# autonomousvision/volsurfs

Measured on AMD Instinct MI355X. Metric: Mrays/s (fwd+bwd) at 800x800, K=5 shells, higher is better.
Workload: dtype f16 (hash features, MLP on MFMA, composite: as the reference), f32 accumulate and I/O

## Files before the change

include/volsurfs_hip.h:

```cpp
#ifndef VOLSURFS_HIP_H
#define VOLSURFS_HIP_H

#include <stdint.h>

#ifdef __cplusplus
extern "C" {
#endif

#define VSA_OK 0
#define VSA_ERR_ARG (-1)
#define VSA_ERR_UNSUPPORTED (-2)

#define VSA_MAX_SHELLS 16

int vsa_version(void);

int vsa_composite_dense_fwd(const float* surfs_rgb, const float* surfs_alpha,
                            const float* rgb_bg, int bg_is_broadcast, float* out_rgb,
                            float* out_rgb_fg, float* out_bg_transmittance, float* out_weights,
                            float* out_surfs_rgb_h, float* out_surfs_alpha_h, int nr_rays,
                            int nr_shells, int carry_f16, void* stream);

int vsa_composite_dense_bwd(const float* surfs_rgb, const float* surfs_alpha,
                            const float* rgb_bg, int bg_is_broadcast, const float* g_rgb,
// ... 92 lines not shown
  void* balance;
  int32_t row_format;
  int32_t grads_zeroed;
  int32_t shared_rgb;
  int32_t shared_alpha;
} vsa_nt_plan;

long long vsa_nt_balance_bytes(void);
int vsa_nt_rebalance(const vsa_nt_plan* plan, void* stream);

int vsa_nt_mark(const vsa_nt_plan* plan, const int32_t* hit_slot, const float* hit_uv,
                const float* face_uvs, int nr_rays, float* tex_uv, uint8_t* marks, void* stream);

int vsa_nt_compact_frame(const vsa_nt_plan* plan, uint8_t* marks, int32_t* slot_of,
                         int32_t* texel_of_slot, float* slot_xy, int32_t* seg_start,
                         int32_t* block_scratch, void* stream);

int vsa_nt_encode_fwd(const vsa_nt_plan* plan, const void* tables_h, const float* slot_xy,
                      const int32_t* seg_start, void* features, void* stream);

int vsa_nt_mlp_fwd(const vsa_nt_plan* plan, const void* weights_h, const void* features,
                   const int32_t* seg_start, uint8_t* texels, void* pre_out, void* stream);

int vsa_nt_encode_mlp_fwd(const vsa_nt_plan* plan, const void* tables_h, const void* weights_h,
                          const float* slot_xy, const int32_t* seg_start, void* features,
                          uint8_t* texels, void* pre_out, void* stream);

int vsa_nt_mlp_bwd(const vsa_nt_plan* plan, const void* weights_h, void* features,
                   const int32_t* seg_start, uint16_t* grad_rows, float* grad_weights,
                   float* dfeat_abs_sum, float weight_grad_scale, void* stream);

int vsa_nt_shade_fwd(const vsa_nt_plan* plan, const int32_t* hit_slot, const float* tex_uv,
                     const float* rays_d, const float* tris, const int32_t* slot_of,
                     const int32_t* seg_start, const uint8_t* texels, int nr_rays,
                     float* surfs_rgb, float* surfs_alpha,
                     float* surfs_normals, float* coeffs_out, float* act_out, void* stream);

int vsa_nt_shade_bwd(const vsa_nt_plan* plan, const int32_t* hit_slot, const float* tex_uv,
                     const float* rays_d, const float* tris, const int32_t* slot_of,
                     const int32_t* seg_start, const uint8_t* texels, int nr_rays,
                     const float* g_surfs_rgb,
                     const float* g_surfs_alpha, float grad_scale, uint16_t* grad_rows,
                     const float* act_in, void* stream);

long long vsa_nt_planes_bytes(const vsa_nt_plan* plan);
int vsa_nt_export_planes(const vsa_nt_plan* plan, const int32_t* slot_of, const int32_t* seg_start,
                         const uint8_t* texels, uint8_t* planes, long long planes_bytes, void* stream);
int vsa_nt_import_planes(const vsa_nt_plan* plan, const uint8_t* planes, long long planes_bytes,
                         const int32_t* slot_of, const int32_t* seg_start, uint8_t* texels, void* stream);

int vsa_nt_encode_bwd(const vsa_nt_plan* plan, const void* dfeatures, const float* dfeat_abs_sum,
                      float grad_scale, const float* slot_xy, const int32_t* seg_start,
                      float* grad_tables, void* stream);

int vsa_nt_encode_bwd_range(const vsa_nt_plan* plan, const void* dfeatures,
                            const float* dfeat_abs_sum, float grad_scale, const float* slot_xy,
                            const int32_t* seg_start, float* grad_tables, int shell_begin,
                            int shell_end, void* stream);

typedef struct vsa_dp_flags vsa_dp_flags;
int vsa_dp_flags_create(int n, vsa_dp_flags** out);
int vsa_dp_flags_destroy(vsa_dp_flags* flags);
int vsa_dp_flags_read(const vsa_dp_flags* flags, uint32_t* host_out);

int vsa_nt_encode_bwd_phased(const vsa_nt_plan* plan, const void* dfeatures,
                             const float* dfeat_abs_sum, float grad_scale, const float* slot_xy,
                             const int32_t* seg_start, float* grad_tables, int n_phases,
                             const int32_t* phase_shell_end, vsa_dp_flags* flags, uint32_t* counters,
                             const uint32_t* epoch, int reserve_cus, void* stream);

int vsa_dp_signal(vsa_dp_flags* flags, int index, uint32_t* epoch, int advance_epoch, void* stream);

int vsa_dp_stream_wait(vsa_dp_flags* flags, int index, uint32_t value, int mode, void* stream);

#define VSA_GRID_MAX_LEVELS 32
typedef struct vsa_grid_plan {
  int32_t n_dims;
  int32_t n_levels;
  int32_t n_features;
  int32_t reserved0;
  float level_scale[VSA_GRID_MAX_LEVELS];
  int32_t level_res[VSA_GRID_MAX_LEVELS];
  int32_t level_size[VSA_GRID_MAX_LEVELS];
  int32_t level_offset[VSA_GRID_MAX_LEVELS + 1];
} vsa_grid_plan;

int vsa_grid_encode_fwd(const vsa_grid_plan* plan, const float* tables, const float* x,
                        int nr_points, float* out, void* stream);
int vsa_grid_encode_bwd(const vsa_grid_plan* plan, const float* x, const float* g_out,
                        int nr_points, float* grad_tables, void* stream);
int vsa_grid_encode_bwd_sliced(const vsa_grid_plan* plan, const float* x, const float* g_out,
                               int nr_points, float* grad_tables, float* workspace, void* stream);
int vsa_grid_encode_bwd_binned_workspace(const vsa_grid_plan* plan, int nr_points,
                                         long long* workspace_floats);
int vsa_grid_encode_bwd_binned(const vsa_grid_plan* plan, const float* x, const float* g_out,
                               int nr_points, float* grad_tables, float* workspace, void* stream);
int vsa_grid_encode_fwd_ld(const vsa_grid_plan* plan, const float* tables, const float* x,
                           int nr_points, float* out, int out_stride, int append_x, void* stream);
int vsa_grid_encode_bwd_ld(const vsa_grid_plan* plan, const float* x, const float* g_out,
                           int g_stride, int nr_points, float* grad_tables, void* stream);
int vsa_grid_encode_bwd_sliced_ld(const vsa_grid_plan* plan, const float* x, const float* g_out,
                                  int g_stride, int nr_points, float* grad_tables, float* workspace,
                                  void* stream);
int vsa_grid_encode_bwd_binned_ld(const vsa_grid_plan* plan, const float* x, const float* g_out,
                                  int g_stride, int nr_points, float* grad_tables, float* workspace,
                                  void* stream);
// ... 551 lines not shown
```

volsurfs_amd/csrc/nt_common.h:

```cpp
#pragma once
#include "common.h"

typedef _Float16 half2_t __attribute__((ext_vector_type(2)));
typedef _Float16 half4_t __attribute__((ext_vector_type(4)));
typedef _Float16 half8_t __attribute__((ext_vector_type(8)));
typedef float float16_t __attribute__((ext_vector_type(16)));

#define NT_DOM_BLOCK 4096

#define NT_FBLOCK 256
__device__ __forceinline__ long long nt_feat_index(const vsa_nt_plan& p, int type, int level,
                                                   int slot) {
  const long long blocks = p.slot_capacity / NT_FBLOCK;
  return (((long long)type * blocks + (slot >> 8)) * p.n_levels + level) * NT_FBLOCK + (slot & 255);
}
__device__ __forceinline__ long long nt_feat_plane_base(const vsa_nt_plan& p, int type, int level) {
  return ((long long)type * (p.slot_capacity / NT_FBLOCK) * p.n_levels + level) * NT_FBLOCK;
}
__device__ __forceinline__ long long nt_feat_in_plane(int n_levels, int slot) {
  return (long long)(slot >> 8) * (n_levels * NT_FBLOCK) + (slot & 255);
}

__host__ __device__ inline int nt_tex_index(int shell, int type, int deg) {
  return (shell * 2 + type) * VSA_NT_MAX_DEG + deg;
// ... 206 lines not shown
    begin = seg_start[sd];
    end = seg_start[sd + 1];
  }
  act = act && end > begin;
  const int units = act ? (end - begin + UNIT - 1) / UNIT : 0;
  const unsigned long long act_mask = __ballot(act);
  const long long pieces = __popcll(act_mask);
  if (pieces == 0) return;
  auto lane_cost = [&](int pl) { return act ? ovh * 16 + units * wt(pl, deg, wtype) : 0; };
  auto plane_cost = [&](int pl) -> long long {
    return (long long)(unsigned)__builtin_amdgcn_readlane(nt_wave_incl_scan(lane_cost(pl)), 63);
  };
  long long total = 0;
  for (int pl = 0; pl < n_planes; ++pl) total += plane_cost(pl);
  long long lo, hi;
  nt_split_range(plan, bal_id, total, lo, hi);
  if (hi <= lo) return;
  long long c0 = 0;
  for (int pl = 0; pl < n_planes && c0 < hi; ++pl) {
    const int cl = lane_cost(pl);
    const int incl = nt_wave_incl_scan(cl);
    const long long pc = (long long)(unsigned)__builtin_amdgcn_readlane(incl, 63);
    if (c0 + pc <= lo) {
      c0 += pc;
      continue;
    }
    const long long t0l = c0 + (long long)(incl - cl) + (long long)ovh * 16;
    const int w = wt(pl, deg, wtype);
    const long long span = (long long)units * w;
    bool hit = act && t0l < hi;
    int ua = 0, ub = 0;
    if (hit) {
      const long long a = lo > t0l ? lo - t0l : 0, b = hi - t0l < span ? hi - t0l : span;
      hit = b > a;
      if (hit) {
        ua = (int)(((unsigned)a + (unsigned)w - 1u) / (unsigned)w);
        ub = (int)(((unsigned)b + (unsigned)w - 1u) / (unsigned)w);
        hit = ub > ua;
      }
    }
    unsigned long long todo = __ballot(hit);
    while (todo) {
      const int j = __ffsll((long long)todo) - 1;
      todo &= todo - 1;
      const int jb = __builtin_amdgcn_readlane(begin, j), je = __builtin_amdgcn_readlane(end, j);
      const int ja = __builtin_amdgcn_readlane(ua, j), jub = __builtin_amdgcn_readlane(ub, j);
      const int first = jb + ja * UNIT;
      const long long lastl = (long long)jb + (long long)jub * UNIT;
      body(pl, j, first, lastl < je ? (int)lastl : je, jb, je);
    }
    c0 += pc;
  }
}
```

volsurfs_amd/csrc/nt_encode.hip:

```cpp
#include <type_traits>

#include "nt_common.h"
#include "nt_enc_common.h"

namespace {

#define NT_ENC_OVH_FH 87
#define NT_ENC_OVH_FD 27
#define NT_ENC_OVH_BH 145
#define NT_ENC_OVH_BD 64
#define NT_ENC_PAIR_W 22
constexpr int ENC_BLOCK = 1024;
constexpr int ENC_UNROLL = 8;
#define ENC_UNROLL_FWD_N 4
constexpr int ENC_UNROLL_FWD = ENC_UNROLL_FWD_N;
constexpr int ENC_UNIT = 256;
constexpr int LDS_ENTRIES = 32768;

constexpr int ENC_PAIR_OFF = 15360;
template <bool HASHED>
__device__ __forceinline__ void nt_encode_fwd_body(
    const vsa_nt_plan& plan, int level0, int n_levels, const half2_t* __restrict__ tables,
    const float2* __restrict__ slot_xy, const int* __restrict__ seg_start,
    half2_t* __restrict__ features, unsigned char* s_raw) {
  half2_t* s_tab = reinterpret_cast<half2_t*>(s_raw);
  const long long n_entries = plan.level_offset[plan.n_levels];
  const int nl = plan.n_levels;
  NT_BAL_BEGIN();
  const bool pair_mode = !HASHED && plan.nr_shells * 2 * VSA_NT_MAX_DEG <= 64;
  auto unit_weight = [&](int pl, int deg, int wtype) {
    const int w = !HASHED || plan.level_scale[level0 + pl] < (float)plan.tex_res[deg] ? 16 : 15;
    return wtype == 2 ? (w * NT_ENC_PAIR_W) >> 4 : w;
  };
  nt_for_each_piece<ENC_UNIT>(plan, seg_start, n_levels, HASHED ? NT_ENC_OVH_FH : NT_ENC_OVH_FD,
                              [&](int pl, int tex, int first, int last, int, int) {
    const int level = level0 + pl;
    const LevelGeom g = level_geom(plan, level);
    const int partner = pair_mode ? nt_pair_partner(plan, tex) : -1;
    const bool pair_fits = (int)g.size <= ENC_PAIR_OFF && ENC_PAIR_OFF + (int)g.size <= LDS_ENTRIES;
    const int tex2 = pair_fits ? partner : -1;
    for (int pass = 0; pass < (partner >= 0 && !pair_fits ? 2 : 1); ++pass) {
    const int tex_p = pass ? partner : tex;
    __syncthreads();
    auto stage = [&](int t, half2_t* dst_h) {
      typedef unsigned u32x4 __attribute__((ext_vector_type(4)));
      const u32x4* src = reinterpret_cast<const u32x4*>(tables + (long long)nt_param_tex(plan, t) * n_entries + plan.level_offset[level]);
      u32x4* dst = reinterpret_cast<u32x4*>(dst_h);
      constexpr int SB = 8;
      const int nvec = (int)(g.size / 4);
      for (int i0 = threadIdx.x; i0 < nvec; i0 += ENC_BLOCK * SB) {
        u32x4 r[SB];
#pragma unroll
        for (int k = 0; k < SB; ++k) {
          const int i = i0 + k * ENC_BLOCK;
          r[k] = src[i < nvec ? i : nvec - 1];
        }
#pragma unroll
        for (int k = 0; k < SB; ++k)
          if (i0 + k * ENC_BLOCK < nvec) dst[i0 + k * ENC_BLOCK] = r[k];
      }
    };
    stage(tex_p, s_tab);
    if (tex2 >= 0) stage(tex2, s_tab + ENC_PAIR_OFF);
    __syncthreads();
    const int type = (tex_p / VSA_NT_MAX_DEG) & 1;
    half2_t* out = features + nt_feat_plane_base(plan, type, level);
    half2_t* out2 = features + nt_feat_plane_base(plan, 1, level);
    const int a_first = first & ~(ENC_UNROLL_FWD - 1);
    auto run = [&](auto reuse_tag, auto pair_tag) {
      constexpr bool REUSE = decltype(reuse_tag)::value;
      constexpr bool PAIR = decltype(pair_tag)::value;
      for (int s0 = a_first + threadIdx.x * ENC_UNROLL_FWD; s0 < last; s0 += ENC_BLOCK * ENC_UNROLL_FWD) {
        float4 xyv[ENC_UNROLL_FWD / 2];
        const float4* xp = reinterpret_cast<const float4*>(slot_xy + s0);
#pragma unroll
        for (int i = 0; i < ENC_UNROLL_FWD / 2; ++i) xyv[i] = xp[i];
        CellRefS cr[ENC_UNROLL_FWD];
        bool fresh[ENC_UNROLL_FWD];
#pragma unroll
        for (int u = 0; u < ENC_UNROLL_FWD; ++u) {
          const float x = (u & 1) ? xyv[u >> 1].z : xyv[u >> 1].x;
          const float y = (u & 1) ? xyv[u >> 1].w : xyv[u >> 1].y;
          cr[u] = cell_ref_s(g, x, y);
          fresh[u] = !REUSE || u == 0 || cr[u].cx != cr[u - 1].cx || cr[u].cy != cr[u - 1].cy;
        }
        half2_t v[ENC_UNROLL_FWD][4], v2[PAIR ? ENC_UNROLL_FWD : 1][4];
#pragma unroll
        for (int u = 0; u < ENC_UNROLL_FWD; ++u) {
// ... 17 lines not shown
            if constexpr (PAIR) {
#pragma unroll
              for (int k = 0; k < 4; ++k) v2[u][k] = v2[u - 1][k];
            }
          }
          unsigned ew[4];
#pragma unroll
          for (int k = 0; k < 4; ++k) ew[k] = __builtin_bit_cast(unsigned, v[u][k]);
          if constexpr (PAIR) {
            half2_t wh[4];
            enc_weights_h(cr[u].w, wh);
            outw[u] = enc_blend_h(ew, wh);
#pragma unroll
            for (int k = 0; k < 4; ++k) ew[k] = __builtin_bit_cast(unsigned, v2[u][k]);
            outw2[u] = enc_blend_h(ew, wh);
          } else
          {
            outw[u] = enc_blend(ew, cr[u].w);
          }
        }
        const long long o_in = nt_feat_in_plane(nl, s0);
        unsigned* op = reinterpret_cast<unsigned*>(out) + o_in;
        unsigned* op2 = reinterpret_cast<unsigned*>(out2) + o_in;
        if (s0 >= first && s0 + ENC_UNROLL_FWD <= last) {
          uint4* o4 = reinterpret_cast<uint4*>(op);
#pragma unroll
          for (int i = 0; i < ENC_UNROLL_FWD / 4; ++i)
            o4[i] = make_uint4(outw[4 * i], outw[4 * i + 1], outw[4 * i + 2], outw[4 * i + 3]);
          if constexpr (PAIR) {
            uint4* p4 = reinterpret_cast<uint4*>(op2);
#pragma unroll
            for (int i = 0; i < ENC_UNROLL_FWD / 4; ++i)
              p4[i] = make_uint4(outw2[4 * i], outw2[4 * i + 1], outw2[4 * i + 2], outw2[4 * i + 3]);
          }
        } else {
#pragma unroll
          for (int u = 0; u < ENC_UNROLL_FWD; ++u)
            if (s0 + u >= first && s0 + u < last) {
              op[u] = outw[u];
              if constexpr (PAIR) op2[u] = outw2[u];
            }
        }
      }
    };
    const bool reuse = g.scale < (float)plan.tex_res[tex % VSA_NT_MAX_DEG];
    if (!HASHED && tex2 >= 0) {
      if (reuse) run(std::true_type{}, std::true_type{});
      else run(std::false_type{}, std::true_type{});
    } else {
      if (reuse) run(std::true_type{}, std::false_type{});
      else run(std::false_type{}, std::false_type{});
    }
    }
  }, 0, 1 << 30, unit_weight, HASHED ? NT_BAL_ENC_FWD_H : NT_BAL_ENC_FWD_D, pair_mode);
  __syncthreads();
  NT_BAL_END(HASHED ? NT_BAL_ENC_FWD_H : NT_BAL_ENC_FWD_D);
}

template <bool HASHED>
__global__ __launch_bounds__(ENC_BLOCK) void nt_encode_fwd_kernel(
    vsa_nt_plan plan, int level0, int n_levels, const half2_t* __restrict__ tables,
    const float2* __restrict__ slot_xy, const int* __restrict__ seg_start,
    half2_t* __restrict__ features) {
  extern __shared__ __attribute__((aligned(16))) unsigned char s_raw[];
  nt_encode_fwd_body<HASHED>(plan, level0, n_levels, tables, slot_xy, seg_start, features, s_raw);
}

__global__ __launch_bounds__(ENC_BLOCK) void nt_encode_fwd_both_kernel(
    vsa_nt_plan plan, int lh, const half2_t* __restrict__ tables,
    const float2* __restrict__ slot_xy, const int* __restrict__ seg_start,
    half2_t* __restrict__ features) {
  extern __shared__ __attribute__((aligned(16))) unsigned char s_raw[];
  nt_encode_fwd_body<false>(plan, 0, lh, tables, slot_xy, seg_start, features, s_raw);
  __syncthreads();
  nt_encode_fwd_body<true>(plan, lh, plan.n_levels - lh, tables, slot_xy, seg_start, features, s_raw);
}

#define NT_ENC_FLUSH_BATCH 8
template <bool HASHED, int NF, bool MERGE>
__device__ __forceinline__ void enc_bwd_piece(
    const vsa_nt_plan& plan, int* s_g, int level, int feat, int tex, int first, int last,
    bool store, const half2_t* __restrict__ dfeatures, const float* __restrict__ dfeat_abs_sum,
    float dscale_inv, const float2* __restrict__ slot_xy, float* __restrict__ grad_tables) {
  const int nl = plan.n_levels;
  const long long n_entries = plan.level_offset[plan.n_levels];
  const LevelGeom g = level_geom(plan, level);
  float S[NF], S_inv[NF];
  bool any = false;
#pragma unroll
  for (int f = 0; f < NF; ++f) {
    const float total = dfeat_abs_sum[tex * 32 + 2 * level + feat + f] * 1.001f;
    S[f] = 0.f, S_inv[f] = 0.f;
    if (total > 0.f) {
      int e;
      frexpf(total, &e);
      S[f] = ldexpf(1.0f, 30 - e);
      S_inv[f] = ldexpf(1.0f, e - 30) * dscale_inv;
      any = true;
    }
  }
  if (!any) return;
  int copies = 1;
  if (!HASHED) {
    while (copies < 32 && (long long)g.size * copies * 2 * NF <= LDS_ENTRIES) copies *= 2;
  }
  const int plane = (int)g.size * copies;
  __syncthreads();
  for (int i = threadIdx.x; i < plane * NF; i += ENC_BLOCK) s_g[i] = 0;
  int* my_g = s_g + (threadIdx.x & (copies - 1)) * g.size;
  const int type = (tex / VSA_NT_MAX_DEG) & 1;
  const unsigned* dFw = reinterpret_cast<const unsigned*>(dfeatures + nt_feat_plane_base(plan, type, level));
  __syncthreads();
  const int a_first = first & ~(ENC_UNROLL - 1);
  constexpr int PD = 1;
  const int s_max = (last - 1) & ~(ENC_UNROLL - 1);
  float4 xyn[PD][ENC_UNROLL / 2];
  uint4 dn[PD][ENC_UNROLL / 4];
  auto request = [&](int s, float4 (&xd)[ENC_UNROLL / 2], uint4 (&dd)[ENC_UNROLL / 4]) {
    const int sc = s < s_max ? s : s_max;
    const float4* xp = reinterpret_cast<const float4*>(slot_xy + sc);
    const uint4* dp = reinterpret_cast<const uint4*>(dFw + nt_feat_in_plane(nl, sc));
#pragma unroll
    for (int i = 0; i < ENC_UNROLL / 2; ++i) xd[i] = xp[i];
#pragma unroll
    for (int i = 0; i < ENC_UNROLL / 4; ++i) dd[i] = dp[i];
  };
#pragma unroll
  for (int d = 0; d < PD; ++d)
// ... 85 lines not shown
      asm volatile("" ::"v"(xyn[d][i].x), "v"(xyn[d][i].y), "v"(xyn[d][i].z), "v"(xyn[d][i].w));
#pragma unroll
    for (int i = 0; i < ENC_UNROLL / 4; ++i)
      asm volatile("" ::"v"(dn[d][i].x), "v"(dn[d][i].y), "v"(dn[d][i].z), "v"(dn[d][i].w));
  }
  __syncthreads();
  float* gt = grad_tables + ((long long)nt_param_tex(plan, tex) * n_entries + plan.level_offset[level]) * 2 + feat;
  constexpr int FB = NT_ENC_FLUSH_BATCH;
  auto plane_sums = [&](int i0, int (&vi)[FB][NF]) {
#pragma unroll
    for (int b = 0; b < FB; ++b) {
      const int i = i0 + b * ENC_BLOCK;
#pragma unroll
      for (int f = 0; f < NF; ++f) {
        int acc = 0;
        if (i < (int)g.size)
          for (int cpy = 0; cpy < copies; ++cpy) acc += s_g[f * plane + cpy * g.size + i];
        vi[b][f] = acc;
      }
    }
  };
  if (store) {
    for (int i0 = threadIdx.x; i0 < (int)g.size; i0 += ENC_BLOCK * FB) {
      int vi[FB][NF];
      plane_sums(i0, vi);
#pragma unroll
      for (int b = 0; b < FB; ++b) {
        const long long i = i0 + b * ENC_BLOCK;
        if constexpr (NF == 2) {
          if ((vi[b][0] | vi[b][1]) != 0)
            *reinterpret_cast<float2*>(&gt[2 * i]) = make_float2((float)vi[b][0] * S_inv[0], (float)vi[b][1] * S_inv[1]);
        } else {
          if (vi[b][0] != 0) gt[2 * i] = (float)vi[b][0] * S_inv[0];
        }
      }
    }
  } else {
    for (int i0 = threadIdx.x; i0 < (int)g.size; i0 += ENC_BLOCK * FB) {
      int vi[FB][NF];
      plane_sums(i0, vi);
#pragma unroll
      for (int b = 0; b < FB; ++b)
#pragma unroll
        for (int f = 0; f < NF; ++f)
          if (vi[b][f] != 0) atomicAdd(&gt[2 * (long long)(i0 + b * ENC_BLOCK) + f], (float)vi[b][f] * S_inv[f]);
    }
  }
}

__device__ __host__ inline bool enc_both_features(const vsa_nt_plan& p, int level, bool hashed) {
  return !hashed && (long long)p.level_size[level] * 2 <= LDS_ENTRIES;
}

template <bool HASHED>
__device__ __forceinline__ void nt_encode_bwd_body(
    const vsa_nt_plan& plan, int level0, int n_levels, int n_planes,
    const half2_t* __restrict__ dfeatures, const float* __restrict__ dfeat_abs_sum,
    float dscale_inv, const float2* __restrict__ slot_xy, const int* __restrict__ seg_start,
    float* __restrict__ grad_tables, int tex_begin, int tex_end, unsigned char* s_raw) {
  int* s_g = reinterpret_cast<int*>(s_raw);
  NT_BAL_BEGIN();
  const bool full_range = tex_begin <= 0 && tex_end >= plan.nr_shells * 2 * VSA_NT_MAX_DEG;
  auto unit_weight = [&](int pl, int deg, int) {
    return !HASHED || plan.level_scale[level0 + (pl >> 1)] < (float)plan.tex_res[deg] ? 16 : 14;
  };
  nt_for_each_piece<ENC_UNIT>(plan, seg_start, n_planes, HASHED ? NT_ENC_OVH_BH : NT_ENC_OVH_BD,
                              [&](int pl, int tex, int first, int last, int seg_begin, int seg_end) {
    int level = level0, r = pl;
    bool both = enc_both_features(plan, level, HASHED);
    while (r >= (both ? 1 : 2)) {
      r -= both ? 1 : 2;
      ++level;
      both = enc_both_features(plan, level, HASHED);
    }
    const bool shared_plane = (((tex / VSA_NT_MAX_DEG) & 1) ? plan.shared_alpha : plan.shared_rgb) != 0;
    const bool store = plan.grads_zeroed != 0 && first == seg_begin && last == seg_end && !shared_plane;
    const bool merge = plan.level_scale[level] < (float)plan.tex_res[tex % VSA_NT_MAX_DEG];
    if (both)
      enc_bwd_piece<HASHED, 2, true>(plan, s_g, level, 0, tex, first, last, store, dfeatures,
                                     dfeat_abs_sum, dscale_inv, slot_xy, grad_tables);
    else if (merge)
      enc_bwd_piece<HASHED, 1, true>(plan, s_g, level, r, tex, first, last, store, dfeatures,
                                     dfeat_abs_sum, dscale_inv, slot_xy, grad_tables);
    else
      enc_bwd_piece<HASHED, 1, false>(plan, s_g, level, r, tex, first, last, store, dfeatures,
                                      dfeat_abs_sum, dscale_inv, slot_xy, grad_tables);
  }, tex_begin, tex_end, unit_weight,
     full_range ? (HASHED ? NT_BAL_ENC_BWD_H : NT_BAL_ENC_BWD_D) : -1);
  __syncthreads();
  if (full_range) { NT_BAL_END(HASHED ? NT_BAL_ENC_BWD_H : NT_BAL_ENC_BWD_D); }
}

template <bool HASHED>
__global__ __launch_bounds__(ENC_BLOCK) void nt_encode_bwd_kernel(
    vsa_nt_plan plan, int level0, int n_levels, int n_planes,
    const half2_t* __restrict__ dfeatures, const float* __restrict__ dfeat_abs_sum,
    float dscale_inv, const float2* __restrict__ slot_xy, const int* __restrict__ seg_start,
    float* __restrict__ grad_tables, int tex_begin, int tex_end) {
  extern __shared__ __attribute__((aligned(16))) unsigned char s_raw[];
  nt_encode_bwd_body<HASHED>(plan, level0, n_levels, n_planes, dfeatures, dfeat_abs_sum, dscale_inv, slot_xy,
                             seg_start, grad_tables, tex_begin, tex_end, s_raw);
}

__global__ __launch_bounds__(ENC_BLOCK) void nt_encode_bwd_both_kernel(
    vsa_nt_plan plan, int lh, int n_planes_dense,
    const half2_t* __restrict__ dfeatures, const float* __restrict__ dfeat_abs_sum,
    float dscale_inv, const float2* __restrict__ slot_xy, const int* __restrict__ seg_start,
    float* __restrict__ grad_tables, int tex_begin, int tex_end) {
  extern __shared__ __attribute__((aligned(16))) unsigned char s_raw[];
  nt_encode_bwd_body<false>(plan, 0, lh, n_planes_dense, dfeatures, dfeat_abs_sum, dscale_inv, slot_xy,
                            seg_start, grad_tables, tex_begin, tex_end, s_raw);
  __syncthreads();
  nt_encode_bwd_body<true>(plan, lh, plan.n_levels - lh, 2 * (plan.n_levels - lh), dfeatures, dfeat_abs_sum,
                           dscale_inv, slot_xy, seg_start, grad_tables, tex_begin, tex_end, s_raw);
}

struct EncPhases {
  int n;
  int shell_end[VSA_MAX_SHELLS];
  unsigned* flag[VSA_MAX_SHELLS];
};

__global__ __launch_bounds__(ENC_BLOCK) void nt_encode_bwd_phased_kernel(
    vsa_nt_plan plan, int lh, int n_planes_dense,
    const half2_t* __restrict__ dfeatures, const float* __restrict__ dfeat_abs_sum,
    float dscale_inv, const float2* __restrict__ slot_xy, const int* __restrict__ seg_start,
    float* __restrict__ grad_tables, EncPhases ph,
    unsigned* __restrict__ counters, const unsigned* __restrict__ epoch) {
  extern __shared__ __attribute__((aligned(16))) unsigned char s_raw[];
  if (lh > 0)
    nt_encode_bwd_body<false>(plan, 0, lh, n_planes_dense, dfeatures, dfeat_abs_sum, dscale_inv, slot_xy,
                              seg_start, grad_tables, 0, 1 << 30, s_raw);
  __syncthreads();
  int shell0 = 0;
  for (int p = 0; p < ph.n; ++p) {
    const int tex_begin = shell0 * 2 * VSA_NT_MAX_DEG, tex_end = ph.shell_end[p] * 2 * VSA_NT_MAX_DEG;
    shell0 = ph.shell_end[p];
    if (lh < plan.n_levels)
      nt_encode_bwd_body<true>(plan, lh, plan.n_levels - lh, 2 * (plan.n_levels - lh), dfeatures, dfeat_abs_sum,
                               dscale_inv, slot_xy, seg_start, grad_tables, tex_begin, tex_end, s_raw);
    __builtin_amdgcn_s_waitcnt(0);
    __syncthreads();
    if (threadIdx.x == 0) {
      __builtin_amdgcn_fence(__ATOMIC_RELEASE, "agent");
      const unsigned done = __hip_atomic_fetch_add(&counters[p], 1u, __ATOMIC_ACQ_REL, __HIP_MEMORY_SCOPE_AGENT);
      if (done == gridDim.x - 1) {
        __hip_atomic_store(&counters[p], 0u, __ATOMIC_RELAXED, __HIP_MEMORY_SCOPE_AGENT);
        __hip_atomic_store(ph.flag[p], *epoch, __ATOMIC_RELEASE, __HIP_MEMORY_SCOPE_SYSTEM);
      }
    }
  }
}

__global__ void dp_signal_kernel(unsigned* __restrict__ flag, unsigned* __restrict__ epoch, int advance) {
  unsigned e = *epoch;
  if (advance) *epoch = ++e;
  __hip_atomic_store(flag, e, __ATOMIC_RELEASE, __HIP_MEMORY_SCOPE_SYSTEM);
}

__global__ void dp_spin_wait_kernel(const unsigned* __restrict__ flag, unsigned value) {
  while ((int)(__hip_atomic_load(flag, __ATOMIC_RELAXED, __HIP_MEMORY_SCOPE_SYSTEM) - value) < 0)
    __builtin_amdgcn_s_sleep(64);
  __builtin_amdgcn_fence(__ATOMIC_ACQUIRE, "");
}

}

static bool level_hashed(const vsa_nt_plan* p, int l) {
  const long long res = p->level_res[l], size = p->level_size[l];
  return !(res <= size && res * res <= size);
}

static int first_hashed_level(const vsa_nt_plan* p) {
  int l = 0;
  while (l < p->n_levels && !level_hashed(p, l)) ++l;
  return l;
}

static int check_levels(const vsa_nt_plan* p) {
  const int lh = first_hashed_level(p);
  for (int l = lh; l < p->n_levels; ++l) {
    if (!level_hashed(p, l)) return VSA_ERR_UNSUPPORTED;
    const int sz = p->level_size[l];
    if ((sz & (sz - 1)) != 0 || sz > LDS_ENTRIES) return VSA_ERR_UNSUPPORTED;
  }
  for (int l = 0; l < lh; ++l)
    if (p->level_size[l] > LDS_ENTRIES) return VSA_ERR_UNSUPPORTED;
  return VSA_OK;
}

static int max_level_size(const vsa_nt_plan* p, int l0, int l1) {
  int m = 0;
  for (int l = l0; l < l1; ++l) m = m > p->level_size[l] ? m : p->level_size[l];
  return m;
}

template <typename K>
static int set_lds_attr(K kernel) {
  VSA_HIP_TRY(hipFuncSetAttribute(reinterpret_cast<const void*>(kernel),
                                  hipFuncAttributeMaxDynamicSharedMemorySize, 159 * 1024));
  return VSA_OK;
}

extern "C" int vsa_nt_encode_fwd(const vsa_nt_plan* plan, const void* tables_h,
                                 const float* slot_xy, const int32_t* seg_start, void* features,
                                 void* stream) {
  if (!plan || !tables_h || !slot_xy || !seg_start || !features) return VSA_ERR_ARG;
  int rc = check_levels(plan);
  if (rc) return rc;
  static bool attr_set = false;
  if (!attr_set) {
    if ((rc = set_lds_attr(nt_encode_fwd_kernel<false>))) return rc;
    if ((rc = set_lds_attr(nt_encode_fwd_kernel<true>))) return rc;
    if ((rc = set_lds_attr(nt_encode_fwd_both_kernel))) return rc;
    attr_set = true;
  }
  const int lh = first_hashed_level(plan);
  const half2_t* tab = reinterpret_cast<const half2_t*>(tables_h);
  const float2* xy = reinterpret_cast<const float2*>(slot_xy);
  half2_t* out = reinterpret_cast<half2_t*>(features);
  int nr_cus = 0;
  if ((rc = vsa_cu_count(&nr_cus))) return rc;
  if (lh > 0 && lh < plan->n_levels) {
    hipLaunchKernelGGL(nt_encode_fwd_both_kernel, dim3(nr_cus), dim3(ENC_BLOCK), (size_t)LDS_ENTRIES * 4,
                       (hipStream_t)stream, *plan, lh, tab, xy, seg_start, out);
    VSA_RETURN_LAUNCH_STATUS();
  }
  if (lh > 0)
    hipLaunchKernelGGL(nt_encode_fwd_kernel<false>, dim3(nr_cus), dim3(ENC_BLOCK),
                       (size_t)LDS_ENTRIES * 4, (hipStream_t)stream, *plan, 0, lh, tab, xy,
                       seg_start, out);
  if (lh < plan->n_levels)
    hipLaunchKernelGGL(nt_encode_fwd_kernel<true>, dim3(nr_cus), dim3(ENC_BLOCK),
                       (size_t)LDS_ENTRIES * 4, (hipStream_t)stream, *plan, lh, plan->n_levels - lh,
                       tab, xy, seg_start, out);
  VSA_RETURN_LAUNCH_STATUS();
}

extern "C" int vsa_nt_encode_bwd(const vsa_nt_plan* plan, const void* dfeatures,
                                 const float* dfeat_abs_sum, float grad_scale,
                                 const float* slot_xy, const int32_t* seg_start,
                                 float* grad_tables, void* stream) {
  if (!plan) return VSA_ERR_ARG;
  return vsa_nt_encode_bwd_range(plan, dfeatures, dfeat_abs_sum, grad_scale, slot_xy, seg_start,
                                 grad_tables, 0, plan->nr_shells, stream);
}

extern "C" int vsa_nt_encode_bwd_range(const vsa_nt_plan* plan, const void* dfeatures,
                                       const float* dfeat_abs_sum, float grad_scale,
                                       const float* slot_xy, const int32_t* seg_start,
                                       float* grad_tables, int shell_begin, int shell_end,
                                       void* stream) {
  if (!plan || !dfeatures || !dfeat_abs_sum || !slot_xy || !seg_start || !grad_tables)
    return VSA_ERR_ARG;
  if (shell_begin < 0 || shell_end > plan->nr_shells || shell_begin > shell_end) return VSA_ERR_ARG;
  if (shell_begin == shell_end) return VSA_OK;
  if ((plan->shared_rgb || plan->shared_alpha) && !(shell_begin == 0 && shell_end == plan->nr_shells)) return VSA_ERR_UNSUPPORTED;
  const int tex_begin = shell_begin * 2 * VSA_NT_MAX_DEG, tex_end = shell_end * 2 * VSA_NT_MAX_DEG;
  if (!(grad_scale > 0.f)) return VSA_ERR_ARG;
  int rc = check_levels(plan);
  if (rc) return rc;
  static bool attr_set = false;
  if (!attr_set) {
    if ((rc = set_lds_attr(nt_encode_bwd_kernel<false>))) return rc;
    if ((rc = set_lds_attr(nt_encode_bwd_kernel<true>))) return rc;
    if ((rc = set_lds_attr(nt_encode_bwd_both_kernel))) return rc;
    attr_set = true;
  }
  const int lh = first_hashed_level(plan);
  const half2_t* dF = reinterpret_cast<const half2_t*>(dfeatures);
  const float2* xy = reinterpret_cast<const float2*>(slot_xy);
  int nr_cus = 0;
  if ((rc = vsa_cu_count(&nr_cus))) return rc;
  if (lh > 0 && lh < plan->n_levels) {
    int n_planes = 0;
    for (int l = 0; l < lh; ++l) n_planes += enc_both_features(*plan, l, false) ? 1 : 2;
    hipLaunchKernelGGL(nt_encode_bwd_both_kernel, dim3(nr_cus), dim3(ENC_BLOCK), (size_t)LDS_ENTRIES * 4,
                       (hipStream_t)stream, *plan, lh, n_planes, dF, dfeat_abs_sum, 1.0f / grad_scale, xy,
                       seg_start, grad_tables, tex_begin, tex_end);
    VSA_RETURN_LAUNCH_STATUS();
  }
  if (lh > 0) {
    int n_planes = 0;
    for (int l = 0; l < lh; ++l) n_planes += enc_both_features(*plan, l, false) ? 1 : 2;
    hipLaunchKernelGGL(nt_encode_bwd_kernel<false>, dim3(nr_cus), dim3(ENC_BLOCK),
                       (size_t)LDS_ENTRIES * 4, (hipStream_t)stream, *plan, 0, lh, n_planes, dF,
                       dfeat_abs_sum, 1.0f / grad_scale, xy, seg_start, grad_tables, tex_begin,
                       tex_end);
  }
  if (lh < plan->n_levels)
    hipLaunchKernelGGL(nt_encode_bwd_kernel<true>, dim3(nr_cus), dim3(ENC_BLOCK),
                       (size_t)LDS_ENTRIES * 4, (hipStream_t)stream, *plan, lh, plan->n_levels - lh,
                       2 * (plan->n_levels - lh), dF, dfeat_abs_sum, 1.0f / grad_scale, xy,
                       seg_start, grad_tables, tex_begin, tex_end);
  VSA_RETURN_LAUNCH_STATUS();
}

struct vsa_dp_flags {
  int n = 0;
  bool signal_memory = false;
  unsigned* word[VSA_MAX_SHELLS + 1] = {};
};

extern "C" int vsa_dp_flags_create(int n, vsa_dp_flags** out) {
  if (!out || n < 1 || n > VSA_MAX_SHELLS + 1) return VSA_ERR_ARG;
  vsa_dp_flags* f = new vsa_dp_flags();
  f->n = n;
  f->signal_memory = true;
  for (int i = 0; i < n; ++i) {
    void* p = nullptr;
    if (f->signal_memory && hipExtMallocWithFlags(&p, 8, hipMallocSignalMemory) != hipSuccess) {
      (void)hipGetLastError();
      f->signal_memory = false;
      for (int j = 0; j < i; ++j) (void)hipFree(f->word[j]);
      i = -1;
      continue;
    }
    if (!f->signal_memory) VSA_HIP_TRY(hipMalloc(&p, 8));
    VSA_HIP_TRY(hipMemset(p, 0, 8));
    f->word[i] = static_cast<unsigned*>(p);
  }
  *out = f;
  return VSA_OK;
}

extern "C" int vsa_dp_flags_destroy(vsa_dp_flags* f) {
  if (!f) return VSA_OK;
  for (int i = 0; i < f->n; ++i) (void)hipFree(f->word[i]);
  delete f;
  return VSA_OK;
}

// ... 71 lines not shown
```

volsurfs_amd/neural_textures.py:

```python
import ctypes
import math
import os

import numpy as np
import torch

from . import _lib

MAX_SHELLS, MAX_DEG, MAX_LEVELS = 16, 4, 16
DOM_BLOCK = 4096
WEIGHTS_PER_TEX = 8192
REBALANCE = os.environ.get("VSA_NT_REBALANCE", "1") != "0"
FUSED_FORWARD = {"0": False, "1": True}.get(os.environ.get("VSA_NT_FUSED", "auto"), "auto")

class Plan(ctypes.Structure):
    _fields_ = [
        ("nr_shells", ctypes.c_int32), ("rgb_degrees", ctypes.c_int32),
        ("alpha_degrees", ctypes.c_int32), ("inner_solid", ctypes.c_int32),
        ("with_alpha_decay", ctypes.c_int32), ("n_levels", ctypes.c_int32),
        ("tex_res", ctypes.c_int32 * MAX_DEG), ("sh_lo", ctypes.c_float * MAX_DEG),
        ("sh_span", ctypes.c_float * MAX_DEG), ("level_scale", ctypes.c_float * MAX_LEVELS),
        ("level_res", ctypes.c_int32 * MAX_LEVELS), ("level_size", ctypes.c_int32 * MAX_LEVELS),
        ("level_offset", ctypes.c_int32 * (MAX_LEVELS + 1)),
        ("dom_off", ctypes.c_int64 * (MAX_SHELLS * MAX_DEG + 1)),
# ... 181 lines not shown
        if self.row_format != 0:
            raise _lib.VolsurfsHipError("baked textures are the 8-bit deploy format: using_sh_quantization=1 only")
        self.compact_all()
        self.evaluate(need_features=False)
        self.baked = True
        return self

    @torch.no_grad()
    def compact_all(self, want_texel_of_slot=True):
        self.marks.zero_()
        for s in range(self.K):
            for d in range(self.D):
                R = self.tex_res[d]
                W = R + 2
                if min(4 * self.max_rays, W * W) < W * W:
                    raise _lib.VolsurfsHipError("bake_all needs a full-capacity bank "
                                                "(max_rays >= NeuralTextureBank.full_capacity_rays)")
                off = int(self.plan.dom_off[s * MAX_DEG + d])
                self.marks[off:off + W * W].view(W, W).fill_(1)
        _lib.call("vsa_nt_compact_frame", ctypes.byref(self.plan), self.marks, self.slot_of,
                  self.texel_of_slot if want_texel_of_slot else None, self.slot_xy, self.seg_start,
                  self.block_scratch, _lib.stream_ptr())

    @torch.no_grad()
    def baked_textures(self):
        dense = self.rows_dense(self.texels)
        out = {}
        for s in range(self.K):
            for d in range(self.D):
                R = self.tex_res[d]
                W, n = R + 2, 2 * d + 1
                off = int(self.plan.dom_off[s * MAX_DEG + d])
                slots = self.slot_of[off:off + W * W].view(W, W)[1:R + 1, 1:R + 1].long()
                rows = dense[slots]
                if self.tex_channels(self.tex_index(s, 0, d)):
                    out[(s, 0, d)] = rows[..., :3 * n].contiguous()
                if self.tex_channels(self.tex_index(s, 1, d)):
                    out[(s, 1, d)] = rows[..., 24:24 + n].contiguous()
        return out

    def tex_uv_only(self, hit_slot, hit_uv, face_uvs):
        K, N = hit_slot.shape
        tex_uv = torch.empty(K, N, 2, device=hit_slot.device)
        _lib.call("vsa_nt_mark", ctypes.byref(self.plan), hit_slot, hit_uv, face_uvs, N, tex_uv,
                  None, _lib.stream_ptr())
        return tex_uv

    def wait_params(self):
        ev = getattr(self, "_params_event", None)
        if ev is not None:
            torch.cuda.current_stream().wait_event(ev)
            self._params_event = None

    def encode(self):
        self.wait_params()
        _lib.call("vsa_nt_encode_fwd", ctypes.byref(self.plan), self.tables_h, self.slot_xy,
                  self.seg_start, self.features, _lib.stream_ptr())
        return self.features

    def features_level_major(self):
        f = self.features.permute(0, 2, 1, 3, 4)
        return f.reshape(2, 16, self.slot_capacity, 2)

    def mlp(self, want_pre=False):
        self.wait_params()
        pre = None
        if want_pre:
            pre = torch.zeros(self.slot_capacity, 32, dtype=torch.float16, device=self.texels.device)
        _lib.call("vsa_nt_mlp_fwd", ctypes.byref(self.plan), self.weights_h, self.features,
                  self.seg_start, self.texels, pre, _lib.stream_ptr())
        return (self.rows_dense(self.texels), pre) if want_pre else self.texels

    def encode_mlp(self, write_features=True, want_pre=False):
        self.wait_params()
        pre = None
        if want_pre:
            pre = torch.zeros(self.slot_capacity, 32, dtype=torch.float16, device=self.texels.device)
        _lib.call("vsa_nt_encode_mlp_fwd", ctypes.byref(self.plan), self.tables_h, self.weights_h,
                  self.slot_xy, self.seg_start, self.features if write_features else None,
                  self.texels, pre, _lib.stream_ptr())
        return (self.rows_dense(self.texels), pre) if want_pre else self.texels

    def evaluate(self, need_features=True):
        if self.row_format == 0 and (FUSED_FORWARD is True or (FUSED_FORWARD == "auto" and not need_features)):
            return self.encode_mlp(write_features=need_features)
        self.encode()
        return self.mlp()

    def rows_dense(self, buf):
        seg = self.seg_start.cpu().tolist()
        dense = torch.zeros(self.slot_capacity, 32, dtype=buf.dtype, device=buf.device)
        for s in range(self.K):
            for d in range(self.D):
                sd, n, q = s * MAX_DEG + d, 2 * d + 1, ROW_QUADS[d]
                a, b = seg[sd], seg[sd + 1]
                r0 = int(self.plan.row_base[sd]) * 4
                rows = buf[r0:r0 + (b - a) * q * 4].view(b - a, q * 4)
                dense[a:b, :3 * n] = rows[:, :3 * n]
                dense[a:b, 24:24 + n] = rows[:, 4 * ALPHA_QUAD[d]:4 * ALPHA_QUAD[d] + n]
        return dense

    def shade(self, hit_slot, tex_uv, rays_d, tris, want_coeffs=False, want_normals=False,
              act_out=None):
        K, N = hit_slot.shape
        dev = hit_slot.device
        rgb = torch.empty(N, K, 3, device=dev)
# ... 121 lines not shown
```

Measured before the change: 269.1.

## Add sibling-group work scheduling for hashed encode levels

```diff
diff --git a/include/volsurfs_hip.h b/include/volsurfs_hip.h
--- a/include/volsurfs_hip.h
+++ b/include/volsurfs_hip.h
@@ -168,6 +168,8 @@
 int vsa_nt_encode_bwd(const vsa_nt_plan* plan, const void* dfeatures, const float* dfeat_abs_sum,
                       float grad_scale, const float* slot_xy, const int32_t* seg_start,
                       float* grad_tables, void* stream);
+
+int vsa_nt_encode_config(int sibling_groups, int grid_override);
 
 int vsa_nt_encode_bwd_range(const vsa_nt_plan* plan, const void* dfeatures,
                             const float* dfeat_abs_sum, float grad_scale, const float* slot_xy,
diff --git a/volsurfs_amd/csrc/nt_common.h b/volsurfs_amd/csrc/nt_common.h
--- a/volsurfs_amd/csrc/nt_common.h
+++ b/volsurfs_amd/csrc/nt_common.h
@@ -282,3 +282,94 @@
     c0 += pc;
   }
 }
+
+__host__ __device__ inline bool nt_sibling_grid_ok(int grid, int G) { return grid > 0 && grid % (8 * G) == 0; }
+
+__host__ __device__ inline void nt_sibling_stretch(int block, int grid, int G, long long total, int& group,
+                                                   int& member, long long& lo, long long& hi) {
+  const int r = block % (8 * G), n_groups = grid / G;
+  group = block / (8 * G) * 8 + r % 8;
+  member = r / 8;
+  lo = total * group / n_groups;
+  hi = total * (group + 1) / n_groups;
+}
+
+__host__ __device__ inline void nt_sibling_share(int member, int G, int n_sib, int& sib, int& ua, int& ub) {
+  const int r = G / n_sib, j = member / n_sib, n = ub - ua;
+  sib = member % n_sib;
+  ub = ua + n * (j + 1) / r;
+  ua = ua + n * j / r;
+}
+
+template <int UNIT, int G, typename Body, typename Weight>
+__device__ __forceinline__ void nt_for_each_sibling_piece(const vsa_nt_plan& plan, const int* __restrict__ seg_start,
+                                                          int n_levels, int ovh, Body&& body, Weight wt) {
+  constexpr int NF = G / 2;
+  const int n_all = plan.nr_shells * 2 * VSA_NT_MAX_DEG;
+  const int lane = threadIdx.x & 63;
+  const int tex = lane;
+  const int deg = tex % VSA_NT_MAX_DEG, type = (tex / VSA_NT_MAX_DEG) & 1, shell = tex / (2 * VSA_NT_MAX_DEG);
+  const bool rgb_act = deg < plan.rgb_degrees, alpha_act = nt_shell_has_alpha(plan, shell) && deg < plan.alpha_degrees;
+  bool act = tex < n_all && (type == 0 ? rgb_act : (alpha_act && !rgb_act));
+  const int n_types = (rgb_act ? 1 : 0) + (alpha_act ? 1 : 0);
+  const int sd = shell * VSA_NT_MAX_DEG + deg;
+  int begin = 0, end = 0;
+  if (act) {
+    begin = seg_start[sd];
+    end = seg_start[sd + 1];
+  }
+  act = act && end > begin;
+  const int units = act ? (end - begin + UNIT - 1) / UNIT : 0;
+  if (__ballot(act) == 0ull) return;
+  auto unit_w = [&](int lvl) {
+    const int w = wt(lvl * NF, deg, type) * n_types * NF / G;
+    return w > 0 ? w : 1;
+  };
+  auto lane_cost = [&](int lvl) { return act ? ovh * 16 + units * unit_w(lvl) : 0; };
+  long long total = 0;
+  for (int lvl = 0; lvl < n_levels; ++lvl)
+    total += (long long)(unsigned)__builtin_amdgcn_readlane(nt_wave_incl_scan(lane_cost(lvl)), 63);
+  int group, member;
+  long long lo, hi;
+  nt_sibling_stretch((int)blockIdx.x, (int)gridDim.x, G, total, group, member, lo, hi);
+  if (hi <= lo) return;
+  long long c0 = 0;
+  for (int lvl = 0; lvl < n_levels && c0 < hi; ++lvl) {
+    const int cl = lane_cost(lvl);
+    const int incl = nt_wave_incl_scan(cl);
+    const long long pc = (long long)(unsigned)__builtin_amdgcn_readlane(incl, 63);
+    if (c0 + pc <= lo) {
+      c0 += pc;
+      continue;
+    }
+    const long long t0l = c0 + (long long)(incl - cl) + (long long)ovh * 16;
+    const int w = unit_w(lvl);
+    const long long span = (long long)units * w;
+    bool hit = act && t0l < hi;
+    int ua = 0, ub = 0;
+    if (hit) {
+      const long long a = lo > t0l ? lo - t0l : 0, b = hi - t0l < span ? hi - t0l : span;
+      hit = b > a;
+      if (hit) {
+        ua = (int)(((unsigned)a + (unsigned)w - 1u) / (unsigned)w);
+        ub = (int)(((unsigned)b + (unsigned)w - 1u) / (unsigned)w);
+        hit = ub > ua;
+      }
+    }
+    unsigned long long todo = __ballot(hit);
+    while (todo) {
+      const int j = __ffsll((long long)todo) - 1;
+      todo &= todo - 1;
+      const int jb = __builtin_amdgcn_readlane(begin, j), je = __builtin_amdgcn_readlane(end, j);
+      const int jn = __builtin_amdgcn_readlane(n_types, j);
+      int sib, ma = __builtin_amdgcn_readlane(ua, j), mb = __builtin_amdgcn_readlane(ub, j);
+      nt_sibling_share(member, G, jn * NF, sib, ma, mb);
+      if (mb <= ma) continue;
+      const int jtex = sib % jn ? j ^ VSA_NT_MAX_DEG : j;
+      const int first = jb + ma * UNIT;
+      const long long lastl = (long long)jb + (long long)mb * UNIT;
+      body(lvl * NF + sib / jn, jtex, first, lastl < je ? (int)lastl : je, jb, je);
+    }
+    c0 += pc;
+  }
+}
diff --git a/volsurfs_amd/csrc/nt_encode.hip b/volsurfs_amd/csrc/nt_encode.hip
--- a/volsurfs_amd/csrc/nt_encode.hip
+++ b/volsurfs_amd/csrc/nt_encode.hip
@@ -9,6 +9,7 @@
 #define NT_ENC_OVH_FD 27
 #define NT_ENC_OVH_BH 145
 #define NT_ENC_OVH_BD 64
+#define NT_ENC_SIBLING_GROUPS 2
 #define NT_ENC_PAIR_W 22
 constexpr int ENC_BLOCK = 1024;
 constexpr int ENC_UNROLL = 8;
@@ -18,7 +19,7 @@
 constexpr int LDS_ENTRIES = 32768;
 
 constexpr int ENC_PAIR_OFF = 15360;
-template <bool HASHED>
+template <bool HASHED, bool SIB = false>
 __device__ __forceinline__ void nt_encode_fwd_body(
     const vsa_nt_plan& plan, int level0, int n_levels, const half2_t* __restrict__ tables,
     const float2* __restrict__ slot_xy, const int* __restrict__ seg_start,
@@ -32,8 +33,7 @@
     const int w = !HASHED || plan.level_scale[level0 + pl] < (float)plan.tex_res[deg] ? 16 : 15;
     return wtype == 2 ? (w * NT_ENC_PAIR_W) >> 4 : w;
   };
-  nt_for_each_piece<ENC_UNIT>(plan, seg_start, n_levels, HASHED ? NT_ENC_OVH_FH : NT_ENC_OVH_FD,
-                              [&](int pl, int tex, int first, int last, int, int) {
+  auto piece = [&](int pl, int tex, int first, int last, int, int) {
     const int level = level0 + pl;
     const LevelGeom g = level_geom(plan, level);
     const int partner = pair_mode ? nt_pair_partner(plan, tex) : -1;
@@ -157,7 +157,12 @@
       else run(std::false_type{}, std::false_type{});
     }
     }
-  }, 0, 1 << 30, unit_weight, HASHED ? NT_BAL_ENC_FWD_H : NT_BAL_ENC_FWD_D, pair_mode);
+  };
+  if constexpr (SIB)
+    nt_for_each_sibling_piece<ENC_UNIT, 2>(plan, seg_start, n_levels, NT_ENC_OVH_FH, piece, unit_weight);
+  else
+    nt_for_each_piece<ENC_UNIT>(plan, seg_start, n_levels, HASHED ? NT_ENC_OVH_FH : NT_ENC_OVH_FD, piece,
+                                0, 1 << 30, unit_weight, HASHED ? NT_BAL_ENC_FWD_H : NT_BAL_ENC_FWD_D, pair_mode);
   __syncthreads();
   NT_BAL_END(HASHED ? NT_BAL_ENC_FWD_H : NT_BAL_ENC_FWD_D);
 }
@@ -171,6 +176,7 @@
   nt_encode_fwd_body<HASHED>(plan, level0, n_levels, tables, slot_xy, seg_start, features, s_raw);
 }
 
+template <bool SIB>
 __global__ __launch_bounds__(ENC_BLOCK) void nt_encode_fwd_both_kernel(
     vsa_nt_plan plan, int lh, const half2_t* __restrict__ tables,
     const float2* __restrict__ slot_xy, const int* __restrict__ seg_start,
@@ -178,7 +184,7 @@
   extern __shared__ __attribute__((aligned(16))) unsigned char s_raw[];
   nt_encode_fwd_body<false>(plan, 0, lh, tables, slot_xy, seg_start, features, s_raw);
   __syncthreads();
-  nt_encode_fwd_body<true>(plan, lh, plan.n_levels - lh, tables, slot_xy, seg_start, features, s_raw);
+  nt_encode_fwd_body<true, SIB>(plan, lh, plan.n_levels - lh, tables, slot_xy, seg_start, features, s_raw);
 }
 
 #define NT_ENC_FLUSH_BATCH 8
@@ -370,7 +376,7 @@
   return !hashed && (long long)p.level_size[level] * 2 <= LDS_ENTRIES;
 }
 
-template <bool HASHED>
+template <bool HASHED, bool SIB = false>
 __device__ __forceinline__ void nt_encode_bwd_body(
     const vsa_nt_plan& plan, int level0, int n_levels, int n_planes,
     const half2_t* __restrict__ dfeatures, const float* __restrict__ dfeat_abs_sum,
@@ -382,8 +388,7 @@
   auto unit_weight = [&](int pl, int deg, int) {
     return !HASHED || plan.level_scale[level0 + (pl >> 1)] < (float)plan.tex_res[deg] ? 16 : 14;
   };
-  nt_for_each_piece<ENC_UNIT>(plan, seg_start, n_planes, HASHED ? NT_ENC_OVH_BH : NT_ENC_OVH_BD,
-                              [&](int pl, int tex, int first, int last, int seg_begin, int seg_end) {
+  auto piece = [&](int pl, int tex, int first, int last, int seg_begin, int seg_end) {
     int level = level0, r = pl;
     bool both = enc_both_features(plan, level, HASHED);
     while (r >= (both ? 1 : 2)) {
@@ -403,8 +408,13 @@
     else
       enc_bwd_piece<HASHED, 1, false>(plan, s_g, level, r, tex, first, last, store, dfeatures,
                                       dfeat_abs_sum, dscale_inv, slot_xy, grad_tables);
-  }, tex_begin, tex_end, unit_weight,
-     full_range ? (HASHED ? NT_BAL_ENC_BWD_H : NT_BAL_ENC_BWD_D) : -1);
+  };
+  if constexpr (SIB)
+    nt_for_each_sibling_piece<ENC_UNIT, 4>(plan, seg_start, n_levels, NT_ENC_OVH_BH, piece, unit_weight);
+  else
+    nt_for_each_piece<ENC_UNIT>(plan, seg_start, n_planes, HASHED ? NT_ENC_OVH_BH : NT_ENC_OVH_BD, piece,
+                                tex_begin, tex_end, unit_weight,
+                                full_range ? (HASHED ? NT_BAL_ENC_BWD_H : NT_BAL_ENC_BWD_D) : -1);
   __syncthreads();
   if (full_range) { NT_BAL_END(HASHED ? NT_BAL_ENC_BWD_H : NT_BAL_ENC_BWD_D); }
 }
@@ -420,6 +430,7 @@
                              seg_start, grad_tables, tex_begin, tex_end, s_raw);
 }
 
+template <bool SIB>
 __global__ __launch_bounds__(ENC_BLOCK) void nt_encode_bwd_both_kernel(
     vsa_nt_plan plan, int lh, int n_planes_dense,
     const half2_t* __restrict__ dfeatures, const float* __restrict__ dfeat_abs_sum,
@@ -429,8 +440,8 @@
   nt_encode_bwd_body<false>(plan, 0, lh, n_planes_dense, dfeatures, dfeat_abs_sum, dscale_inv, slot_xy,
                             seg_start, grad_tables, tex_begin, tex_end, s_raw);
   __syncthreads();
-  nt_encode_bwd_body<true>(plan, lh, plan.n_levels - lh, 2 * (plan.n_levels - lh), dfeatures, dfeat_abs_sum,
-                           dscale_inv, slot_xy, seg_start, grad_tables, tex_begin, tex_end, s_raw);
+  nt_encode_bwd_body<true, SIB>(plan, lh, plan.n_levels - lh, 2 * (plan.n_levels - lh), dfeatures, dfeat_abs_sum,
+                                dscale_inv, slot_xy, seg_start, grad_tables, tex_begin, tex_end, s_raw);
 }
 
 struct EncPhases {
@@ -513,6 +524,31 @@
   return m;
 }
 
+struct EncConfig {
+  int sibling_groups, grid_override;
+};
+static EncConfig& enc_config() {
+  static EncConfig cfg{NT_ENC_SIBLING_GROUPS, 0};
+  return cfg;
+}
+extern "C" int vsa_nt_encode_config(int sibling_groups, int grid_override) {
+  if (sibling_groups < 0 || sibling_groups > 3 || grid_override < 0 || grid_override > 4096) return VSA_ERR_ARG;
+  enc_config() = EncConfig{sibling_groups, grid_override};
+  return VSA_OK;
+}
+static int enc_grid(int* grid) {
+  if (enc_config().grid_override > 0) {
+    *grid = enc_config().grid_override;
+    return VSA_OK;
+  }
+  return vsa_cu_count(grid);
+}
+static bool enc_siblings(const vsa_nt_plan* p, int grid, int G) {
+  const int mode = enc_config().sibling_groups;
+  const bool on = mode == 1 || mode == (G == 4 ? 2 : 3);
+  return on && nt_sibling_grid_ok(grid, G) && p->nr_shells * 2 * VSA_NT_MAX_DEG <= 64;
+}
+
 template <typename K>
 static int set_lds_attr(K kernel) {
   VSA_HIP_TRY(hipFuncSetAttribute(reinterpret_cast<const void*>(kernel),
@@ -530,7 +566,8 @@
   if (!attr_set) {
     if ((rc = set_lds_attr(nt_encode_fwd_kernel<false>))) return rc;
     if ((rc = set_lds_attr(nt_encode_fwd_kernel<true>))) return rc;
-    if ((rc = set_lds_attr(nt_encode_fwd_both_kernel))) return rc;
+    if ((rc = set_lds_attr(nt_encode_fwd_both_kernel<false>))) return rc;
+    if ((rc = set_lds_attr(nt_encode_fwd_both_kernel<true>))) return rc;
     attr_set = true;
   }
   const int lh = first_hashed_level(plan);
@@ -538,10 +575,14 @@
   const float2* xy = reinterpret_cast<const float2*>(slot_xy);
   half2_t* out = reinterpret_cast<half2_t*>(features);
   int nr_cus = 0;
-  if ((rc = vsa_cu_count(&nr_cus))) return rc;
+  if ((rc = enc_grid(&nr_cus))) return rc;
   if (lh > 0 && lh < plan->n_levels) {
-    hipLaunchKernelGGL(nt_encode_fwd_both_kernel, dim3(nr_cus), dim3(ENC_BLOCK), (size_t)LDS_ENTRIES * 4,
-                       (hipStream_t)stream, *plan, lh, tab, xy, seg_start, out);
+    if (enc_siblings(plan, nr_cus, 2))
+      hipLaunchKernelGGL(nt_encode_fwd_both_kernel<true>, dim3(nr_cus), dim3(ENC_BLOCK), (size_t)LDS_ENTRIES * 4,
+                         (hipStream_t)stream, *plan, lh, tab, xy, seg_start, out);
+    else
+      hipLaunchKernelGGL(nt_encode_fwd_both_kernel<false>, dim3(nr_cus), dim3(ENC_BLOCK), (size_t)LDS_ENTRIES * 4,
+                         (hipStream_t)stream, *plan, lh, tab, xy, seg_start, out);
     VSA_RETURN_LAUNCH_STATUS();
   }
   if (lh > 0)
@@ -582,20 +623,26 @@
   if (!attr_set) {
     if ((rc = set_lds_attr(nt_encode_bwd_kernel<false>))) return rc;
     if ((rc = set_lds_attr(nt_encode_bwd_kernel<true>))) return rc;
-    if ((rc = set_lds_attr(nt_encode_bwd_both_kernel))) return rc;
+    if ((rc = set_lds_attr(nt_encode_bwd_both_kernel<false>))) return rc;
+    if ((rc = set_lds_attr(nt_encode_bwd_both_kernel<true>))) return rc;
     attr_set = true;
   }
   const int lh = first_hashed_level(plan);
   const half2_t* dF = reinterpret_cast<const half2_t*>(dfeatures);
   const float2* xy = reinterpret_cast<const float2*>(slot_xy);
   int nr_cus = 0;
-  if ((rc = vsa_cu_count(&nr_cus))) return rc;
+  if ((rc = enc_grid(&nr_cus))) return rc;
   if (lh > 0 && lh < plan->n_levels) {
     int n_planes = 0;
     for (int l = 0; l < lh; ++l) n_planes += enc_both_features(*plan, l, false) ? 1 : 2;
-    hipLaunchKernelGGL(nt_encode_bwd_both_kernel, dim3(nr_cus), dim3(ENC_BLOCK), (size_t)LDS_ENTRIES * 4,
-                       (hipStream_t)stream, *plan, lh, n_planes, dF, dfeat_abs_sum, 1.0f / grad_scale, xy,
-                       seg_start, grad_tables, tex_begin, tex_end);
+    if (shell_begin == 0 && shell_end == plan->nr_shells && enc_siblings(plan, nr_cus, 4))
+      hipLaunchKernelGGL(nt_encode_bwd_both_kernel<true>, dim3(nr_cus), dim3(ENC_BLOCK), (size_t)LDS_ENTRIES * 4,
+                         (hipStream_t)stream, *plan, lh, n_planes, dF, dfeat_abs_sum, 1.0f / grad_scale, xy,
+                         seg_start, grad_tables, tex_begin, tex_end);
+    else
+      hipLaunchKernelGGL(nt_encode_bwd_both_kernel<false>, dim3(nr_cus), dim3(ENC_BLOCK), (size_t)LDS_ENTRIES * 4,
+                         (hipStream_t)stream, *plan, lh, n_planes, dF, dfeat_abs_sum, 1.0f / grad_scale, xy,
+                         seg_start, grad_tables, tex_begin, tex_end);
     VSA_RETURN_LAUNCH_STATUS();
   }
   if (lh > 0) {
diff --git a/volsurfs_amd/neural_textures.py b/volsurfs_amd/neural_textures.py
--- a/volsurfs_amd/neural_textures.py
+++ b/volsurfs_amd/neural_textures.py
@@ -257,6 +257,10 @@
             torch.cuda.current_stream().wait_event(ev)
             self._params_event = None
 
+    @staticmethod
+    def encode_config(sibling_groups, grid_override=0):
+        _lib.call("vsa_nt_encode_config", int(sibling_groups), int(grid_override))
+
     def encode(self):
         self.wait_params()
         _lib.call("vsa_nt_encode_fwd", ctypes.byref(self.plan), self.tables_h, self.slot_xy,
```

After: 274.1, median of 6. 1.8% higher.
